# Pablete1234/parquet-floor

Measured on AMD Instinct MI355X. Metric: decoded GB/s + rows/s (node), lineitem-shape Snappy+dict, 1/2/4/8 GPUs, higher is better.
Workload: dtype u8; 1 GPU; lineitem SF1 x1 (6001215 rows x 1, 16 cols, 6 row groups of 1Mi rows), Snappy + dictionary, device-resident; row_groups_per_rank=6, compressed_page_bytes_rank0=217870360

## Files before the change

parquet-floor_amd/csrc/pf_internal.h:

```cpp
#pragma once
#include <stdint.h>

#ifdef __HIPCC__
#define PF_HD __host__ __device__
#else
#define PF_HD
#endif

namespace pf {

struct Int2 {
    int x, y;
};

struct PfOpts {
    int exec = 5;
    bool ba_fused = true;
    bool page_null = false;
    int null_stagger = 0;
    bool nest_timeout = false;
    uint32_t null_dcap = 0;
    unsigned debug_skip = 0;
    int force_serial = 0;
    int force_redo = 0;
    bool zc = true;
    bool dl_kernel = true;
    bool h2d_kernel = false;
    int h2d_grid = 256;
    bool dl_stream = true;
    bool dl_prio = false;
    bool debug_plan = false;
    int64_t nest_seg = 0;
    bool nest_seg_set = false;
    bool dbp_par = true;
    bool bloom_first = true;
    bool flat_dstr = true;
    int fix_shift = 1;
};

constexpr uint32_t FBLK = 4096;
constexpr uint32_t BA_TILE = 8192;
constexpr uint64_t BA_SHORT = 48;
constexpr uint32_t STICKY_DICT = 64u << 10;
constexpr uint32_t SNAP_RB = 128;
constexpr uint32_t SNAP_WIN = 64 * SNAP_RB;
constexpr uint32_t SNAP_WWORDS = SNAP_WIN / 32;
constexpr uint32_t SNAP_BLOCK = 65536;

struct SnapWin {
    uint32_t entry;
    uint32_t exit;
    uint32_t out;
    uint32_t flags;
};

struct SnapEnt {
    uint32_t pos;
    uint32_t out;
};
// ... 19 lines not shown
    uint8_t* ddst;
    uint32_t dlo;
    uint32_t dgran;
    uint32_t dflags;
    uint32_t lit;
};

struct ZstdJob {
    const uint8_t* src;
    uint8_t* dst;
    uint32_t src_len;
    uint32_t dst_len;
    int32_t page;
    int32_t chunk;
    uint32_t exact;
    uint32_t produced;
};
constexpr int ZSTD_GRID = 512;
constexpr uint32_t ZSTD_LIT_MAX = 128u << 10;
PF_HD inline uint32_t zstd_lit_stride(uint32_t max_dst) {
    return ((max_dst < ZSTD_LIT_MAX ? max_dst : ZSTD_LIT_MAX) + 255u) / 256u * 256u + 256u;
}

enum : int32_t { DONE_FIXED = 1, DONE_FLAT = 2, DONE_NULL = 4, DONE_PAGE = 8, DONE_DSTR = 16 };

enum : int32_t { DIRECT_NONE = 0, DIRECT_VALUES = 1, DIRECT_INPLACE = 2 };

struct DevPage {
    const uint8_t* body;
    const uint8_t* lvl;
    uint32_t body_len;
    uint32_t rep_len;
    uint32_t def_len;
    int32_t chunk;
    int32_t flags;
    int32_t encoding;
    int32_t def_enc;
    int32_t rep_enc;
    int32_t num_values;
    int32_t done;
    int64_t entry_start;
    int64_t n_slots;
    int64_t n_values;
    int64_t n_rows;
    int64_t n_chars;
    int64_t slot_start;
    int64_t value_start;
// ... 206 lines not shown
```

parquet-floor_amd/csrc/pf_launch.h:

```cpp
#pragma once
#include <hip/hip_runtime.h>

#include "pf_internal.h"
#include "pfloor.h"

namespace pf {

void launch_snappy_serial(const SnappyJob* d_jobs, int n_jobs, const int* d_fallback, DevChunkResult* d_res, hipStream_t s);
void launch_snappy_parse(const SnappyJob* d_jobs, int n_jobs, const int2* d_wins, int n_wins, SnapWin* d_win, SnapEnt* d_ent,
                         uint32_t* d_lane_out, uint32_t* d_splits, int* d_fb, int max_nwin, hipStream_t s);
void launch_snappy_exec(const SnappyJob* d_jobs, int n_jobs, const int2* d_pieces, int n_pieces, uint32_t* d_splits, int* d_fb,
                        DevChunkResult* d_res, int exec, hipStream_t s);
void launch_snappy(const SnappyJob* d_jobs, int n_jobs, const int2* d_wins, int n_wins, SnapWin* d_win, SnapEnt* d_ent,
                   uint32_t* d_lane_out, const int2* d_pieces, int n_pieces, uint32_t* d_splits, int* d_fb,
                   DevChunkResult* d_res, int max_nwin, int exec, hipStream_t s);

void launch_zstd(ZstdJob* d_jobs, const int* d_order, int n_jobs, uint8_t* d_lit, uint32_t lit_stride, DevChunkResult* d_res,
                 hipStream_t s);

void launch_snappy_head(SnappyJob* d_jobs, int n_jobs, DevPage* d_pages, const DevChunk* d_chunks, int* d_fb,
                        const DevChunkResult* d_res, hipStream_t st);
void launch_snappy_litcopy(const SnappyJob* d_jobs, const int* d_list, int n, const int* d_fb, hipStream_t st);

void launch_ba(BaJob* d_jobs, int n_jobs, const int2* d_tiles, int n_tiles, DevChunkResult* d_res, hipStream_t st,
               bool short_values);

void launch_runs(const DevChunk* d_chunks, DevPage* d_pages, const int* d_list, int n, DevChunkResult* d_res, hipStream_t st);
void launch_lvl(const DevChunk* d_chunks, DevPage* d_pages, const int* d_list, int n, DevChunkResult* d_res, hipStream_t st,
                bool page_null, NullCaps nc);
void launch_count_flat(const DevChunk* d_chunks, DevPage* d_pages, const int* d_list, int n, int n_flat, const int2* d_dblk,
                       int n_dblk, DevChunkResult* d_res, BaJob* d_bajobs, hipStream_t st);
void launch_flat(const DevChunk* d_chunks, DevPage* d_pages, const int* d_list, int nfix, int n, int n4, int n8, int* d_fbq,
                 const int2* d_dblk, int n_dblk, DevChunkResult* d_res, hipStream_t st, NullCaps nc, int stagger);

void launch_nest_lvl(const DevChunk* d_chunks, DevPage* d_pages, const int* d_list, int n, int max_nwin, DevChunkResult* d_res,
                     hipStream_t st, bool force_timeout);
void launch_count(const DevChunk* d_chunks, DevPage* d_pages, const int* d_list, int n, DevChunkResult* d_res, BaJob* d_bajobs,
                  hipStream_t st, int idle_grid);
void launch_nest_count(const DevChunk* d_chunks, DevPage* d_pages, const int* d_list, int n, const int2* d_segs, int n_segs,
                       DevChunkResult* d_res, hipStream_t st);
void launch_scan(DevChunk* d_chunks, DevPage* d_pages, const int* d_list, int n, DevChunkResult* d_res, uint8_t* arena,
                 uint64_t cap, unsigned long long* used, hipStream_t st);
void launch_decode(const DevChunk* d_chunks, DevPage* d_pages, const int* d_list, int n, int n_first, DevChunkResult* d_res,
                   hipStream_t st, int idle_grid);
void launch_nest_decode(const DevChunk* d_chunks, DevPage* d_pages, const int2* d_segs, int n_segs, DevChunkResult* d_res,
                        hipStream_t st);

void launch_delta(const DevChunk* d_chunks, DevPage* d_pages, const int* d_list, int n, int max_dbp_nwin, DevChunkResult* d_res,
                  hipStream_t st);
void launch_dlen(const DevChunk* d_chunks, DevPage* d_pages, const int* d_list, int n, DevChunkResult* d_res, hipStream_t st);
void launch_dba_chars(const DevChunk* d_chunks, DevPage* d_pages, const int* d_list, int n, DevChunkResult* d_res, hipStream_t st);

void launch_window(const DevChunk* d_chunks, const DevChunkResult* d_res, const DevWin* d_wins, DevWinRes* d_wres, int n_wins,
                   int copy_grid, const uint8_t* chars_base, uint8_t* wchars_base, int64_t out_delta, int64_t bits_delta,
                   hipStream_t st);

// ... 10 lines not shown
```

parquet-floor_amd/csrc/pf_pages.hip:

```cpp
#include <hip/hip_runtime.h>

#include "pf_dstr_ids.h"
#include "pf_launch.h"
#include "pf_pages.h"
#include "pf_snappy_par.h"

namespace pf {

#ifdef PF_STAMPS
__device__ unsigned long long pf_pstamps[16];
#define PSTAMP(i, v) atomicAdd(&pf_pstamps[i], (unsigned long long)(v))
extern "C" int pf_debug_pstamps(unsigned long long* out, int n, int reset) {
    if (hipMemcpyFromSymbol(out, HIP_SYMBOL(pf_pstamps), sizeof(unsigned long long) * (n < 16 ? n : 16)) != hipSuccess) return -1;
    if (reset) {
        unsigned long long z[16] = {};
        if (hipMemcpyToSymbol(HIP_SYMBOL(pf_pstamps), z, sizeof z) != hipSuccess) return -1;
    }
    return 0;
}
#else
#define PSTAMP(i, v) ((void)0)
#endif

#ifndef PF_FT
// ... 32 lines not shown
    }
    const uint32_t ne = uint32_t(pg.num_values);
    const int id_bw = int(s.val[0]);
    if (tid == 0) {
        s_allp = ck.max_def == 0 ? 1 : (s.def_rle ? all_present(s.def, s.def_n, bit_width(ck.max_def), ne, uint32_t(ck.max_def)) : 0);
    } else if (tid >= 64) {
        __shared__ RunWalk s_st;
        int nr = 0;
        uint32_t cov = 0;
        const int rr = wave_walk_runs(s.val + 1, s.val_n - 1, id_bw, 0, ne, R, RUN_CAP, nr, cov, s_st, RunWalk{0, 0});
        if (tid == 64) { s_res = rr; s_nr = nr; s_cov = cov; }
    }
    __syncthreads();
    const int nr = s_nr;
    if (s_res == 2) {
        if (tid == 0) { T[2] = 0; T[3] = 0; }
        return;
    }
    for (int i = tid; i < nr; i += 128) {
        T[4 + 2 * i] = R[i].first | (R[i].packed << 31);
        T[5 + 2 * i] = R[i].data;
    }
    if (tid == 0) { T[0] = uint32_t(nr); T[1] = s_cov; T[2] = 1u; T[3] = s_allp ? 1u : 0u; }
}

__device__ __forceinline__ bool count_dict_page(const DevPage& pg, const DevChunk& ck, const Sections& s) {
    const uint32_t* T = pg.runtab;
    return T != nullptr && T[3] == 1u && T[0] <= uint32_t(RUN_CAP) && T[1] >= uint32_t(pg.num_values) && ck.dict_len &&
           s.val_n > 0 && flat_block_chars(pg) != nullptr;
}
constexpr uint64_t BC_BAD = ~0ull;

__global__ __launch_bounds__(NT) void k_count_dict(const DevChunk* __restrict__ chunks, DevPage* pages,
                                                   const int2* __restrict__ blocks, DevChunkResult* res) {
    __shared__ Run R[RUN_CAP];
    __shared__ uint32_t s_len[DSTR_CAP];
    __shared__ unsigned long long s_acc;
    const int2 pb = blocks[blockIdx.x];
    DevPage& pg = pages[pb.x];
    const DevChunk& ck = chunks[pg.chunk];
    const int tid = threadIdx.x;
    if (res[pg.chunk].status != 0 || ck.max_rep != 0 || ck.ptype != 6 || !is_dict_enc(pg.encoding)) return;
    Sections s;
    if (!page_sections(pg, ck, s) || !count_dict_page(pg, ck, s)) return;
    const uint32_t ne = uint32_t(pg.num_values);
    const uint32_t b0 = uint32_t(pb.y) * FBLK;
// ... 544 lines not shown
                const uint32_t m = uint32_t((hi - lo >= 32 ? 0xffffffffull : ((1ull << (hi - lo)) - 1ull)) << (lo & 31));
                if (lo == (wd << 5) && hi == ((wd + 1) << 5)) vw[wd] = m;
                else atomicOr(vw + wd, m);
            }
        }
        if (__syncthreads_or(bad)) return 1;
    }
    return 0;
}

__device__ __forceinline__ bool flat_fixed_block(FixedLds& S, const DevChunk* __restrict__ chunks, DevPage* pages, const int2 pbk,
                                 DevChunkResult* res) {
    if (pbk.x < 0) return true;
    const int pi = pbk.x;
    const uint32_t blk = uint32_t(pbk.y) & 0x0fffffffu;
    const uint32_t bsz = FBLK << (uint32_t(pbk.y) >> 28);
    DevPage& pg = pages[pi];
    const DevChunk& ck = chunks[pg.chunk];
    const int tid = threadIdx.x;
    const int* jfb = pg.jfb;
    const bool dval = pg.direct == DIRECT_VALUES;
    const int jf = jfb != nullptr ? *jfb : FB_WHOLE + 1;
    const int done = pg.done;
    if (done & DONE_DSTR) return true;
    if ((res[pg.chunk].status != 0) | (ck.max_rep != 0) | (ck.ptype == 6) | ((done & DONE_NULL) != 0)) return false;
    if (dval & (jf <= FB_WHOLE)) {
        const uint32_t ne = uint32_t(pg.num_values), e_begin = blk * bsz;
        if (e_begin >= ne && blk > 0) return true;
        const uint32_t e_end = min(ne, e_begin + bsz);
        if (ck.max_def > 0 && ck.validity && e_end > e_begin) {
            const uint64_t b0 = uint64_t(pg.entry_start) + e_begin, b1 = uint64_t(pg.entry_start) + e_end;
            uint32_t* vw = reinterpret_cast<uint32_t*>(ck.validity);
            for (uint64_t wd = (b0 >> 5) + threadIdx.x; wd <= ((b1 - 1) >> 5); wd += NT) {
                const uint64_t lo = max(b0, wd << 5), hi = min(b1, (wd + 1) << 5);
                const uint32_t m = uint32_t((hi - lo >= 32 ? 0xffffffffull : ((1ull << (hi - lo)) - 1ull)) << (lo & 31));
                if (lo == (wd << 5) && hi == ((wd + 1) << 5)) vw[wd] = m;
                else atomicOr(vw + wd, m);
            }
        }
        if (threadIdx.x == 0) {
            if (ck.needs_count == 0)
                atomicAdd(reinterpret_cast<unsigned long long*>(&res[pg.chunk].num_values), (unsigned long long)(e_end - e_begin));
            atomicOr(&pg.done, DONE_FIXED);
        }
        return true;
    }
    Sections s;
// ... 406 lines not shown
struct DstrLds {
    uint32_t rt[2 * RUN_CAP];
    uint32_t dpl[DSTR_CAP];
    u32x4 dict[DSTR_DICT / 16 + 2];
    u32x4 win[DSTR_WIN / 16 + 2];
    uint32_t scan_tmp[NT / 64];
    uint32_t wlo[NT / 64], whi[NT / 64];
};
#ifdef PF_DIAG
__device__ unsigned long long pf_dstr_counts[2];
extern "C" int pf_debug_dstr_counts(unsigned long long* out, int reset) {
    if (hipMemcpyFromSymbol(out, HIP_SYMBOL(pf_dstr_counts), sizeof(unsigned long long) * 2) != hipSuccess) return -1;
    if (reset) {
        const unsigned long long z[2] = {0, 0};
        if (hipMemcpyToSymbol(HIP_SYMBOL(pf_dstr_counts), z, sizeof z) != hipSuccess) return -1;
    }
    return 0;
}
#define DSTR_COUNT(i) (threadIdx.x == 0 ? (void)atomicAdd(&pf_dstr_counts[i], 1ull) : (void)0)
#else
#define DSTR_COUNT(i) ((void)0)
#endif

__device__ __forceinline__ u32x4 ld16_within(uintptr_t a, uintptr_t beg, uintptr_t end) {
    if (a >= beg && a + 16u <= end) return *reinterpret_cast<const PF_GLOBAL u32x4*>(a);
    uint32_t q[4] = {0, 0, 0, 0};
    #pragma unroll
    for (uint32_t b = 0; b < 16u; b++)
        if (a + b >= beg && a + b < end) q[b >> 2] |= uint32_t(*reinterpret_cast<const PF_GLOBAL uint8_t*>(a + b)) << (8 * (b & 3));
    return u32x4{q[0], q[1], q[2], q[3]};
}

template <int LEAD>
__device__ __forceinline__ void store_offs16(int32_t* p, const uint32_t (&o)[16]) {
    #pragma unroll
    for (int k = 0; k < LEAD; k++) p[k] = int32_t(o[k]);
    #pragma unroll
    for (int k = LEAD; k + 4 <= 16; k += 4) *reinterpret_cast<u32x4*>(p + k) = u32x4{o[k], o[k + 1], o[k + 2], o[k + 3]};
    #pragma unroll
    for (int k = LEAD + (16 - LEAD) / 4 * 4; k < 16; k++) p[k] = int32_t(o[k]);
}

__global__ __launch_bounds__(NT, PF_DSTR_OCC) void k_flat_dstr(const DevChunk* __restrict__ chunks, DevPage* pages,
                                                            const int2* __restrict__ blocks, DevChunkResult* res) {
    __shared__ DstrLds S;
    const int2 pb = blocks[blockIdx.x];
    const int pi = pb.x;
    const uint32_t blk = uint32_t(pb.y);
    DevPage& pg = pages[pi];
    const DevChunk& ck = chunks[pg.chunk];
    const int tid = threadIdx.x;
    const uint32_t ne = uint32_t(pg.num_values);
    const uint32_t b0 = blk * FBLK;
    if (blk > 0 && b0 >= ne) return;
    bool ok = (res[pg.chunk].status == 0) & (ck.max_rep == 0) & (ck.ptype == 6) & is_dict_enc(pg.encoding) & (pg.counted == 1) &
// ... 8 lines not shown
        const DevPage& dp = pages[ck.dict_page];
        dend = reinterpret_cast<uintptr_t>(dp.body) + dp.body_len;
        ok = dend > dbeg && dend - dbeg <= uintptr_t(DSTR_DICT);
    }
    if (!ok) {
        if (blk == 0) DSTR_COUNT(1);
        return;
    }
    const uint32_t b1 = min(ne, b0 + FBLK);
    const uint32_t* T = pg.runtab;
    const uint32_t nr = T[0], cov = T[1];
    const uint32_t dn = uint32_t(ck.dict_n), dbytes = uint32_t(dend - dbeg);
    const int id_bw = int(s.val[0]);
    const uint8_t* ids = s.val + 1;
    const uint64_t ids_n = s.val_n - 1;
    const uint64_t bc_blk = blk > 0 ? flat_block_chars(pg)[blk] : 0ull;
    int bad = 0;
    uint32_t mylo = 0xffffffffu, myhi = 0u;
    if (uint32_t(tid) < nr) {
        const uint32_t f = T[4 + 2 * tid], d = T[5 + 2 * tid];
        const uint32_t nf = uint32_t(tid) + 1 < nr ? (T[6 + 2 * tid] & 0x7fffffffu) : cov;
        S.rt[2 * tid] = f;
        S.rt[2 * tid + 1] = d;
        const uint32_t first = f & 0x7fffffffu;
        const uint32_t a = max(first, b0), z = min(nf, b1);
        if ((f >> 31) && a < z) {
            mylo = uint32_t((uint64_t(d) + uint64_t(a - first) * uint64_t(id_bw)) >> 3);
            myhi = uint32_t((uint64_t(d) + uint64_t(z - first) * uint64_t(id_bw) + 7u) >> 3);
        }
    }
    const uint32_t doff = uint32_t(dbeg & 15u);
    if (uint32_t(tid) < dn) {
        const uint32_t pos = gptr(ck.dict_pos)[tid], len = gptr(ck.dict_len)[tid];
        bad = (len > DSTR_LMAX) | (pos > dbytes) | (len > dbytes - min(pos, dbytes));
        S.dpl[tid] = (doff + pos) | (len << 16);
    }
    for (uint32_t c = tid; c < (doff + dbytes + 15u) / 16u; c += NT) S.dict[c] = ld16_within(dbeg - doff + 16u * c, dbeg, dend);
    #pragma unroll
    for (int d = 32; d >= 1; d >>= 1) {
        mylo = min(mylo, uint32_t(__shfl_xor(mylo, d, 64)));
        myhi = max(myhi, uint32_t(__shfl_xor(myhi, d, 64)));
    }
    if ((tid & 63) == 0) { S.wlo[tid >> 6] = mylo; S.whi[tid >> 6] = myhi; }
    if (__syncthreads_or(bad)) {
        if (blk == 0) DSTR_COUNT(1);
        return;
    }
    uint32_t lo = 0xffffffffu, hi = 0u;
    #pragma unroll
    for (int w = 0; w < NT / 64; w++) { lo = min(lo, S.wlo[w]); hi = max(hi, S.whi[w]); }
    const uintptr_t ibeg = reinterpret_cast<uintptr_t>(ids), iend = ibeg + ids_n;
    const uintptr_t ia0 = (ibeg + (lo < hi ? lo : 0u)) & ~uintptr_t(15);
    const uint32_t inb = lo < hi ? (uint32_t(ibeg + hi - ia0) + 8u + 15u) & ~15u : 0u;
    const bool ilds = inb > 0 && inb <= uint32_t(sizeof(S.win));
    if (ilds) {
        for (uint32_t c = tid; c < inb / 16u; c += NT) S.win[c] = ld16_within(ia0 + 16u * c, ibeg, iend);
        __syncthreads();
    }
    const int64_t bias = ilds ? 8 * (int64_t(ibeg) - int64_t(ia0)) : 0;
    const uint32_t* const wl = reinterpret_cast<const uint32_t*>(S.win);
    const auto W = [&](uint32_t w) -> uint32_t {
        if (ilds) return wl[w];
        return ld32le(ids, uint64_t(w) * 4u, ids_n);
    };
    const uint32_t e0 = b0 + 16u * uint32_t(tid);
    const uint32_t n = e0 < b1 ? min(16u, b1 - e0) : 0u;
    uint32_t pl[16];
    uint32_t lsum = 0;
    {
        uint32_t id[16];
        dstr_ids16(S.rt, nr, cov, e0, n, id_bw, bias, W, id);
        #pragma unroll
        for (uint32_t k = 0; k < 16; k++) {
            pl[k] = 0;
            if (k >= n) continue;
            if (id[k] >= dn) { bad = 1; continue; }
            pl[k] = S.dpl[id[k]];
            lsum += pl[k] >> 16;
        }
    }
    uint32_t tot;
    const uint32_t lo_c = block_excl_scan<NT>(lsum, S.scan_tmp, tot);
// ... 48 lines not shown
            uint32_t v = my0;
            #pragma unroll
            for (uint32_t k = 0; k < 16; k++) {
                const uint32_t len = pl[k] >> 16, pos = pl[k] & 0xffffu;
                const uint32_t s0 = max(v, w0), s1 = min(v + len, w1);
                for (uint32_t b = s0; b < s1; b++) w8[b - w0] = d8[pos + (b - v)];
                v += len;
            }
        }
        __syncthreads();
        for (uint32_t ci = tid; ci < (w1 - w0 + 15u) / 16u; ci += NT) {
            const uint32_t vp = w0 + 16u * ci;
            if (vp >= a0c && vp + 16u <= vend) {
                *reinterpret_cast<PF_GLOBAL u32x4*>(g0 + vp) = S.win[ci];
            } else {
                for (uint32_t b = 0; b < 16u; b++)
                    if (vp + b >= a0c && vp + b < vend) reinterpret_cast<uint8_t*>(g0 + vp)[b] = w8[16u * ci + b];
            }
        }
    }
    if (tid == 0) {
        atomicOr(&pg.done, DONE_DSTR | DONE_FLAT);
        DSTR_COUNT(0);
    }
}

#ifndef PF_FLAT_OCC
#define PF_FLAT_OCC 5
#endif
__global__ __launch_bounds__(NT, PF_FLAT_OCC) void k_flat_all(const DevChunk* __restrict__ chunks, DevPage* pages,
                                                 const int2* __restrict__ blocks, int n, const int* __restrict__ fbq,
                                                 DevChunkResult* res) {
    __shared__ union FlatAllLds {
        FixedLds f;
        FlatLds g;
    } S;
    if (int(blockIdx.x) >= n) {
        const int nq = fbq[0], g = int(gridDim.x) - n;
        for (int i = int(blockIdx.x) - n; i < nq; i += g) {
            const int2 pq = reinterpret_cast<const int2*>(fbq + 4)[i];
            if (!flat_fixed_block(S.f, chunks, pages, pq, res)) {
                __syncthreads();
                flat_block(S.g, chunks, pages, pq, res);
            }
            __syncthreads();
        }
// ... 358 lines not shown

#ifndef PF_NTN
#define PF_NTN 256
#endif
constexpr int NTN = PF_NTN;
constexpr int NEPT = FBLK / NTN;
static_assert(NEPT % 4 == 0 && NEPT <= 16, "k_flat_null's stores and present masks");
struct NullLds {
    uint2 drun[LT_BLOCK_RUNS + 1];
    uint2 vrun[RUN_CAP + 1];
    uint32_t vbits[FBLK / 32 + 2];
    uint32_t scan_tmp[NTN / 64];
};
__device__ __forceinline__ uint32_t rl_first(uint2 r) { return r.x & 0x7fffffffu; }
__device__ __forceinline__ int rl_find(const uint2* runs, int nr, uint32_t i) {
    int lo = 0, hi = nr;
    while (hi - lo > 1) {
        const int mid = (lo + hi) >> 1;
        if (rl_first(runs[mid]) <= i) lo = mid; else hi = mid;
    }
    return lo;
}


template <int W> struct WidthType { using type = uint64_t; };
template <> struct WidthType<4> { using type = uint32_t; };

template <int W>
__global__ __launch_bounds__(NTN) void k_flat_null(const DevChunk* __restrict__ chunks, DevPage* pages,
                                                   const int2* __restrict__ blocks, DevChunkResult* res, NullCaps nc,
                                                   int stagger, int* fbq) {
    using VT = typename WidthType<W>::type;
    __shared__ __attribute__((aligned(16))) NullLds S;
    extern __shared__ __attribute__((aligned(16))) uint64_t DYN[];
    uint32_t* const s_dst = reinterpret_cast<uint32_t*>(DYN);
    uint32_t* const s_ist = s_dst + (nc.dcap + 32u) / 4u;
    uint64_t* const DL = reinterpret_cast<uint64_t*>(s_ist + (nc.icap + 32u) / 4u);
    const uint32_t dlds = nc.dlds;
    const int2 pbk = blocks[blockIdx.x];
#ifdef PF_DIAG
    if (stagger && pbk.y > 0)
        for (int i = 0; i < stagger; i++) __builtin_amdgcn_s_sleep(127);
#else
    (void)stagger;
#endif
    if (pbk.x < 0) return;
#ifdef PF_STAMPS
    unsigned long long t_ph = __builtin_amdgcn_s_memtime(), t_beg = t_ph;
#define NSTAMP(i) { const unsigned long long t_ = __builtin_amdgcn_s_memtime(); if (threadIdx.x == 0) PSTAMP(i, t_ - t_ph); t_ph = t_; }
// ... 565 lines not shown
#endif

void launch_count_flat(const DevChunk* d_chunks, DevPage* d_pages, const int* d_list, int n, int n_flat, const int2* d_dblk,
                       int n_dblk, DevChunkResult* d_res, BaJob* d_bajobs, hipStream_t st) {
    if (n <= 0) return;
    if (n_dblk > 0) hipLaunchKernelGGL(k_count_dict, dim3(n_dblk), dim3(NT), 0, st, d_chunks, d_pages, d_dblk, d_res);
    if (n_flat > 0) hipLaunchKernelGGL(k_count_flat, dim3(n_flat), dim3(NT), 0, st, d_chunks, d_pages, d_list, d_res, d_bajobs);
}
void launch_runs(const DevChunk* d_chunks, DevPage* d_pages, const int* d_list, int n, DevChunkResult* d_res,
                 hipStream_t st) {
    if (n > 0) hipLaunchKernelGGL(k_runs, dim3(n), dim3(128), 0, st, d_chunks, d_pages, d_list, d_res);
}
void launch_lvl(const DevChunk* d_chunks, DevPage* d_pages, const int* d_list, int n, DevChunkResult* d_res,
                hipStream_t st, bool page_null, NullCaps nc) {
    if (n <= 0) return;
#ifdef PF_DIAG
    if (page_null) hipLaunchKernelGGL(k_page_null, dim3(n), dim3(PN_NT), 0, st, d_chunks, d_pages, d_list, d_res);
#else
    (void)page_null;
#endif
    hipLaunchKernelGGL(k_lvl, dim3(n), dim3(LT_NT), 0, st, d_chunks, d_pages, d_list, d_res, nc.dcap, nc.icap);
}
void launch_flat(const DevChunk* d_chunks, DevPage* d_pages, const int* d_list, int nfix, int n, int n4, int n8, int* d_fbq,
                 const int2* d_dblk, int n_dblk, DevChunkResult* d_res, hipStream_t st, NullCaps nc, int stagger) {
    const int2* blocks = reinterpret_cast<const int2*>(d_list);
    const size_t dyn = size_t(nc.dcap) + 32u + nc.icap + 32u + nc.dlds;
    if (n4 > 0)
        hipLaunchKernelGGL(k_flat_null<4>, dim3(n4), dim3(NTN), dyn, st, d_chunks, d_pages, blocks + nfix + n, d_res, nc, stagger, d_fbq);
    if (n8 > 0)
        hipLaunchKernelGGL(k_flat_null<8>, dim3(n8), dim3(NTN), dyn, st, d_chunks, d_pages, blocks + nfix + n + n4, d_res, nc, stagger,
                           d_fbq);
    if (nfix > 0) hipLaunchKernelGGL(k_flat_fixed, dim3(nfix), dim3(NT), 0, st, d_chunks, d_pages, blocks, d_res, d_fbq);
    if (n_dblk > 0) hipLaunchKernelGGL(k_flat_dstr, dim3(n_dblk), dim3(NT), 0, st, d_chunks, d_pages, d_dblk, d_res);
    const int nq = nfix + n4 + n8;
    const int nqw = nq < 32 ? nq : 32;
    if (n + nqw > 0)
        hipLaunchKernelGGL(k_flat_all, dim3(n + nqw), dim3(NT), 0, st, d_chunks, d_pages, blocks + nfix, n, d_fbq, d_res);
}

}
```

parquet-floor_amd/csrc/pf_runtime.hip:

```cpp
#include <hip/hip_runtime.h>

#include <algorithm>
#include <chrono>
#include <cstdio>
#include <cstdlib>
#include <cstring>
#include <memory>
#include <mutex>
#include <string>
#include <vector>

#include "pf_ctx.h"
#include "pf_host.h"
#include "pf_launch.h"
#include "pf_plan.h"
#include "pf_snappy_par.h"
#include "pfloor.h"

using namespace pf;

static_assert(sizeof(Int2) == sizeof(int2) && alignof(Int2) <= alignof(int2), "the planner's pairs are the kernels' int2");

namespace {

// ... 112 lines not shown
    if (!(skip & 8u)) launch_runs(d_chunks, d_pages, list(L_RUNS), len(L_RUNS), d_res, st);
    NullCaps ncaps = p.null_caps;
    if (ctx->opts.null_dcap) ncaps.dcap = ctx->opts.null_dcap;
    if (!(skip & 8u)) launch_lvl(d_chunks, d_pages, list(L_LVL), len(L_LVL), d_res, st, ctx->opts.page_null, ncaps);
    launch_dlen(d_chunks, d_pages, list(L_DLEN), len(L_DLEN), d_res, st);
    EVREC(ctx, ctx->ev[6], st);
    launch_nest_lvl(d_chunks, d_pages, list(L_NEST), n_nest, p.max_nwin, d_res, st, ctx->opts.nest_timeout);
    if (!(skip & 16u)) {
        launch_count_flat(d_chunks, d_pages, list(L_COUNT), len(L_COUNT), p.n_count_flat, pairs(L_CDICT), len(L_CDICT) / 2,
                          d_res, d_bajobs, st);
        launch_count(d_chunks, d_pages, list(L_COUNT), len(L_COUNT), d_res, d_bajobs, st, COUNT_IDLE_GRID);
    }
    launch_nest_count(d_chunks, d_pages, list(L_NEST), n_nest, pairs(L_NSEG), n_nseg, d_res, st);
    if (!(skip & 4u))
        launch_ba(d_bajobs + p.n_ba_dict, n_ba - p.n_ba_dict, d_batiles + p.n_ba_dict_tiles, n_bt - p.n_ba_dict_tiles,
                  d_res, st, p.ba_short_data && ctx->opts.ba_fused);
    EVREC(ctx, ctx->ev[7], st);
    launch_scan(d_chunks, d_pages, list(L_SCAN), len(L_SCAN), d_res, static_cast<uint8_t*>(ctx->d_chars.p),
                ctx->d_chars.cap, used, st);
    EVREC(ctx, ctx->ev[8], st);
    if (!(skip & 32u))
        launch_flat(d_chunks, d_pages, list(L_FLAT), p.n_flat_fixed, p.n_flat_all, p.n_null4, p.n_null8,
                    reinterpret_cast<int*>(meta + p.off_nfbq), pairs(L_CDICT), ctx->opts.flat_dstr ? len(L_CDICT) / 2 : 0, d_res, st,
                    ncaps, ctx->opts.null_stagger);
    EVREC(ctx, ctx->ev[9], st);
    if (!(skip & 64u)) launch_decode(d_chunks, d_pages, list(L_DECODE), len(L_DECODE), p.n_decode_first, d_res, st, DECODE_IDLE_GRID);
    launch_nest_decode(d_chunks, d_pages, pairs(L_NSEG), n_nseg, d_res, st);
    launch_dba_chars(d_chunks, d_pages, list(L_DBA), len(L_DBA), d_res, st);
    EVREC(ctx, ctx->ev[10], st);
    const WinLayout& wl = ctx->win_lay;
    const bool windowed = !ctx->wins.empty();
    DevWinRes* d_wres = windowed ? reinterpret_cast<DevWinRes*>(static_cast<uint8_t*>(ctx->d_win.p) + wl.res_off) : nullptr;
    if (windowed) {
        EVREC(ctx, ctx->ev_win[0], st);
        launch_window(d_chunks, d_res, static_cast<DevWin*>(ctx->d_win.p), d_wres, int(ctx->wins.size()), ctx->win_grid,
                      static_cast<const uint8_t*>(ctx->d_chars.p), static_cast<uint8_t*>(ctx->d_wchars.p), ctx->twin.out,
                      ctx->twin.bits, st);
        EVREC(ctx, ctx->ev_win[1], st);
        HIPCHK(ctx, hipMemcpyAsync(static_cast<uint8_t*>(ctx->h_win.p) + wl.res_off, d_wres, wl.res_bytes, hipMemcpyDeviceToHost, st));
    }
    if (ctx->filtered()) {
        EVREC(ctx, ctx->ev_sel[0], st);
        launch_filter(d_chunks, d_res, d_wres, ctx->sel, ctx->n_chunks, ctx->sel_lay.grid, static_cast<const uint8_t*>(ctx->d_chars.p),
                      static_cast<uint8_t*>(ctx->d_wchars.p), ctx->twin.out, ctx->twin.bits, st);
        EVREC(ctx, ctx->ev_sel[1], st);
        HIPCHK(ctx, hipMemcpyAsync(ctx->h_sel.p, ctx->d_sel.p, ctx->sel_lay.o_up, hipMemcpyDeviceToHost, st));
    }
// ... 110 lines not shown
    o.null_dcap = uint32_t(std::max(0, num("PF_NULL_DCAP", 0))) & ~15u;
    o.null_stagger = num("PF_DEBUG_NULL_STAGGER", o.null_stagger);
    if (const char* e = std::getenv("PF_DEBUG_SKIP")) {
        const char* names[] = {"parse", "exec", "ba", "levels", "count", "flat", "decode"};
        for (int i = 0; i < 7; i++)
            if (std::strstr(e, names[i])) o.debug_skip |= 1u << i;
    }
    o.force_serial = num("PF_DEBUG_FORCE_SERIAL", o.force_serial);
    o.force_redo = num("PF_DEBUG_FORCE_REDO", o.force_redo);
    o.zc = on("PF_ZC", o.zc);
    o.dl_kernel = on("PF_DL_KERNEL", o.dl_kernel);
    o.dl_stream = on("PF_DL_STREAM", o.dl_stream);
    o.h2d_kernel = on("PF_H2D_KERNEL", o.h2d_kernel);
    o.h2d_grid = std::max(1, num("PF_H2D_GRID", o.h2d_grid));
    o.dl_prio = on("PF_DL_PRIO", o.dl_prio);
    o.debug_plan = on("PF_DEBUG_PLAN", o.debug_plan);
    if (const char* e = std::getenv("PF_NEST_SEG")) {
        o.nest_seg = std::atoll(e);
        o.nest_seg_set = true;
    }
    o.dbp_par = on("PF_DBP_PAR", o.dbp_par);
    o.bloom_first = on("PF_BLOOM_FIRST", o.bloom_first);
    o.flat_dstr = on("PF_FLAT_DSTR", o.flat_dstr);
    const int fb = num("PF_FIX_BLK", 8192);
    o.fix_shift = fb >= 16384 ? 2 : (fb >= 8192 ? 1 : 0);
}
#endif

int ctx_init(pf_ctx* ctx, pf_ctx* peer) {
#ifdef PF_DIAG
    opts_from_env(ctx->opts);
#endif
    HIPCHK(nullptr, hipSetDevice(ctx->device));
    if (peer) {
        ctx->streams = peer->streams;
    } else {
        ctx->streams = std::make_shared<Streams>();
        ctx->streams->device = ctx->device;
        HIPCHK(nullptr, hipStreamCreateWithFlags(&ctx->streams->stream, hipStreamNonBlocking));
    }
    ctx->stream = ctx->streams->stream;
    ctx->zc = ctx->opts.zc;
    HIPCHK(nullptr, hipEventCreateWithFlags(&ctx->ev_done, hipEventDisableTiming));
    HIPCHK(nullptr, hipEventCreateWithFlags(&ctx->ev_copy, hipEventDisableTiming));
    HIPCHK(nullptr, hipEventCreateWithFlags(&ctx->ev_dl, hipEventDisableTiming));
    for (auto& e : ctx->ev) HIPCHK(nullptr, hipEventCreate(&e));
// ... 777 lines not shown
```

Baseline: 392.9 decoded GB/s.

## Add dedicated dictionary-gather kernel for fixed-width dict pages using run tables

Adds k_flat_dfix, launched before k_flat_fixed, which decodes dictionary-encoded 4/8-byte fixed-width pages. It uses the precomputed run table, stages the dictionary and the needed slice of the id stream in LDS, gathers values and writes them with aligned 16-byte stores. Pages it finishes are marked DONE_DFIX so the generic fixed kernel skips them. The aim is to cut the global-memory gathers and scattered stores of the generic path. In exchange it adds another launch and an LDS footprint that may limit occupancy, and pages that fail its checks still fall back to the old path.

```diff
diff --git a/parquet-floor_amd/csrc/pf_internal.h b/parquet-floor_amd/csrc/pf_internal.h
--- a/parquet-floor_amd/csrc/pf_internal.h
+++ b/parquet-floor_amd/csrc/pf_internal.h
@@ -35,6 +35,7 @@
     bool dbp_par = true;
     bool bloom_first = true;
     bool flat_dstr = true;
+    bool flat_dfix = true;
     int fix_shift = 1;
 };
 
@@ -100,7 +101,7 @@
     return ((max_dst < ZSTD_LIT_MAX ? max_dst : ZSTD_LIT_MAX) + 255u) / 256u * 256u + 256u;
 }
 
-enum : int32_t { DONE_FIXED = 1, DONE_FLAT = 2, DONE_NULL = 4, DONE_PAGE = 8, DONE_DSTR = 16 };
+enum : int32_t { DONE_FIXED = 1, DONE_FLAT = 2, DONE_NULL = 4, DONE_PAGE = 8, DONE_DSTR = 16, DONE_DFIX = 32 };
 
 enum : int32_t { DIRECT_NONE = 0, DIRECT_VALUES = 1, DIRECT_INPLACE = 2 };
 
diff --git a/parquet-floor_amd/csrc/pf_launch.h b/parquet-floor_amd/csrc/pf_launch.h
--- a/parquet-floor_amd/csrc/pf_launch.h
+++ b/parquet-floor_amd/csrc/pf_launch.h
@@ -31,7 +31,8 @@
 void launch_count_flat(const DevChunk* d_chunks, DevPage* d_pages, const int* d_list, int n, int n_flat, const int2* d_dblk,
                        int n_dblk, DevChunkResult* d_res, BaJob* d_bajobs, hipStream_t st);
 void launch_flat(const DevChunk* d_chunks, DevPage* d_pages, const int* d_list, int nfix, int n, int n4, int n8, int* d_fbq,
-                 const int2* d_dblk, int n_dblk, DevChunkResult* d_res, hipStream_t st, NullCaps nc, int stagger);
+                 const int2* d_dblk, int n_dblk, DevChunkResult* d_res, hipStream_t st, NullCaps nc, int stagger,
+                 bool dfix);
 
 void launch_nest_lvl(const DevChunk* d_chunks, DevPage* d_pages, const int* d_list, int n, int max_nwin, DevChunkResult* d_res,
                      hipStream_t st, bool force_timeout);
diff --git a/parquet-floor_amd/csrc/pf_pages.hip b/parquet-floor_amd/csrc/pf_pages.hip
--- a/parquet-floor_amd/csrc/pf_pages.hip
+++ b/parquet-floor_amd/csrc/pf_pages.hip
@@ -78,6 +78,54 @@
         T[5 + 2 * i] = R[i].data;
     }
     if (tid == 0) { T[0] = uint32_t(nr); T[1] = s_cov; T[2] = 1u; T[3] = s_allp ? 1u : 0u; }
+}
+
+__device__ __forceinline__ u32x4 ld16_within(uintptr_t a, uintptr_t beg, uintptr_t end) {
+    if (a >= beg && a + 16u <= end) return *reinterpret_cast<const PF_GLOBAL u32x4*>(a);
+    uint32_t q[4] = {0, 0, 0, 0};
+    #pragma unroll
+    for (uint32_t b = 0; b < 16u; b++)
+        if (a + b >= beg && a + b < end) q[b >> 2] |= uint32_t(*reinterpret_cast<const PF_GLOBAL uint8_t*>(a + b)) << (8 * (b & 3));
+    return u32x4{q[0], q[1], q[2], q[3]};
+}
+
+__device__ __forceinline__ void run_id_bytes(uint32_t f, uint32_t d, uint32_t nf, uint32_t b0, uint32_t b1, int id_bw,
+                                             uint32_t& lo, uint32_t& hi) {
+    lo = 0xffffffffu;
+    hi = 0u;
+    const uint32_t first = f & 0x7fffffffu;
+    const uint32_t a = max(first, b0), z = min(nf, b1);
+    if ((f >> 31) && a < z) {
+        lo = uint32_t((uint64_t(d) + uint64_t(a - first) * uint64_t(id_bw)) >> 3);
+        hi = uint32_t((uint64_t(d) + uint64_t(z - first) * uint64_t(id_bw) + 7u) >> 3);
+    }
+}
+__device__ __forceinline__ void id_range_publish(uint32_t mylo, uint32_t myhi, uint32_t* wlo, uint32_t* whi) {
+    #pragma unroll
+    for (int d = 32; d >= 1; d >>= 1) {
+        mylo = min(mylo, uint32_t(__shfl_xor(mylo, d, 64)));
+        myhi = max(myhi, uint32_t(__shfl_xor(myhi, d, 64)));
+    }
+    if ((threadIdx.x & 63) == 0) { wlo[threadIdx.x >> 6] = mylo; whi[threadIdx.x >> 6] = myhi; }
+}
+enum : int { ID_NONE = 0, ID_STAGED = 1, ID_BIG = 2 };
+__device__ __forceinline__ int id_stage_load(u32x4* win, uint32_t cap, const uint32_t* wlo, const uint32_t* whi,
+                                              const uint8_t* ids, uint64_t ids_n, int64_t& bias) {
+    uint32_t lo = 0xffffffffu, hi = 0u;
+    #pragma unroll
+    for (int w = 0; w < NT / 64; w++) { lo = min(lo, wlo[w]); hi = max(hi, whi[w]); }
+    lo = __builtin_amdgcn_readfirstlane(lo);
+    hi = __builtin_amdgcn_readfirstlane(hi);
+    const uintptr_t ibeg = reinterpret_cast<uintptr_t>(ids), iend = ibeg + ids_n;
+    const uintptr_t ia0 = (ibeg + (lo < hi ? lo : 0u)) & ~uintptr_t(15);
+    const uint32_t inb = lo < hi ? (uint32_t(ibeg + hi - ia0) + 8u + 15u) & ~15u : 0u;
+    const bool ilds = inb > 0 && inb <= cap;
+    if (ilds) {
+        for (uint32_t c = threadIdx.x; c < inb / 16u; c += NT) win[c] = ld16_within(ia0 + 16u * c, ibeg, iend);
+        __syncthreads();
+    }
+    bias = ilds ? 8 * (int64_t(ibeg) - int64_t(ia0)) : 0;
+    return ilds ? ID_STAGED : (inb > 0 ? ID_BIG : ID_NONE);
 }
 
 __device__ __forceinline__ bool count_dict_page(const DevPage& pg, const DevChunk& ck, const Sections& s) {
@@ -668,7 +716,7 @@
     const bool dval = pg.direct == DIRECT_VALUES;
     const int jf = jfb != nullptr ? *jfb : FB_WHOLE + 1;
     const int done = pg.done;
-    if (done & DONE_DSTR) return true;
+    if (done & (DONE_DSTR | DONE_DFIX)) return true;
     if ((res[pg.chunk].status != 0) | (ck.max_rep != 0) | (ck.ptype == 6) | ((done & DONE_NULL) != 0)) return false;
     if (dval & (jf <= FB_WHOLE)) {
         const uint32_t ne = uint32_t(pg.num_values), e_begin = blk * bsz;
@@ -1121,15 +1169,6 @@
 #define DSTR_COUNT(i) ((void)0)
 #endif
 
-__device__ __forceinline__ u32x4 ld16_within(uintptr_t a, uintptr_t beg, uintptr_t end) {
-    if (a >= beg && a + 16u <= end) return *reinterpret_cast<const PF_GLOBAL u32x4*>(a);
-    uint32_t q[4] = {0, 0, 0, 0};
-    #pragma unroll
-    for (uint32_t b = 0; b < 16u; b++)
-        if (a + b >= beg && a + b < end) q[b >> 2] |= uint32_t(*reinterpret_cast<const PF_GLOBAL uint8_t*>(a + b)) << (8 * (b & 3));
-    return u32x4{q[0], q[1], q[2], q[3]};
-}
-
 template <int LEAD>
 __device__ __forceinline__ void store_offs16(int32_t* p, const uint32_t (&o)[16]) {
     #pragma unroll
@@ -1184,12 +1223,7 @@
         const uint32_t nf = uint32_t(tid) + 1 < nr ? (T[6 + 2 * tid] & 0x7fffffffu) : cov;
         S.rt[2 * tid] = f;
         S.rt[2 * tid + 1] = d;
-        const uint32_t first = f & 0x7fffffffu;
-        const uint32_t a = max(first, b0), z = min(nf, b1);
-        if ((f >> 31) && a < z) {
-            mylo = uint32_t((uint64_t(d) + uint64_t(a - first) * uint64_t(id_bw)) >> 3);
-            myhi = uint32_t((uint64_t(d) + uint64_t(z - first) * uint64_t(id_bw) + 7u) >> 3);
-        }
+        run_id_bytes(f, d, nf, b0, b1, id_bw, mylo, myhi);
     }
     const uint32_t doff = uint32_t(dbeg & 15u);
     if (uint32_t(tid) < dn) {
@@ -1198,28 +1232,13 @@
         S.dpl[tid] = (doff + pos) | (len << 16);
     }
     for (uint32_t c = tid; c < (doff + dbytes + 15u) / 16u; c += NT) S.dict[c] = ld16_within(dbeg - doff + 16u * c, dbeg, dend);
-    #pragma unroll
-    for (int d = 32; d >= 1; d >>= 1) {
-        mylo = min(mylo, uint32_t(__shfl_xor(mylo, d, 64)));
-        myhi = max(myhi, uint32_t(__shfl_xor(myhi, d, 64)));
-    }
-    if ((tid & 63) == 0) { S.wlo[tid >> 6] = mylo; S.whi[tid >> 6] = myhi; }
+    id_range_publish(mylo, myhi, S.wlo, S.whi);
     if (__syncthreads_or(bad)) {
         if (blk == 0) DSTR_COUNT(1);
         return;
     }
-    uint32_t lo = 0xffffffffu, hi = 0u;
-    #pragma unroll
-    for (int w = 0; w < NT / 64; w++) { lo = min(lo, S.wlo[w]); hi = max(hi, S.whi[w]); }
-    const uintptr_t ibeg = reinterpret_cast<uintptr_t>(ids), iend = ibeg + ids_n;
-    const uintptr_t ia0 = (ibeg + (lo < hi ? lo : 0u)) & ~uintptr_t(15);
-    const uint32_t inb = lo < hi ? (uint32_t(ibeg + hi - ia0) + 8u + 15u) & ~15u : 0u;
-    const bool ilds = inb > 0 && inb <= uint32_t(sizeof(S.win));
-    if (ilds) {
-        for (uint32_t c = tid; c < inb / 16u; c += NT) S.win[c] = ld16_within(ia0 + 16u * c, ibeg, iend);
-        __syncthreads();
-    }
-    const int64_t bias = ilds ? 8 * (int64_t(ibeg) - int64_t(ia0)) : 0;
+    int64_t bias;
+    const bool ilds = id_stage_load(S.win, uint32_t(sizeof(S.win)), S.wlo, S.whi, ids, ids_n, bias) == ID_STAGED;
     const uint32_t* const wl = reinterpret_cast<const uint32_t*>(S.win);
     const auto W = [&](uint32_t w) -> uint32_t {
         if (ilds) return wl[w];
@@ -1314,6 +1333,221 @@
     if (tid == 0) {
         atomicOr(&pg.done, DONE_DSTR | DONE_FLAT);
         DSTR_COUNT(0);
+    }
+}
+
+#ifndef PF_DFIX_LDS
+#define PF_DFIX_LDS 20480
+#endif
+#ifndef PF_DFIX_OCC
+#define PF_DFIX_OCC 5
+#endif
+#ifndef PF_DFIX_H4
+#define PF_DFIX_H4 8
+#endif
+#ifndef PF_DFIX_H8
+#define PF_DFIX_H8 4
+#endif
+static_assert(16 % PF_DFIX_H4 == 0 && PF_DFIX_H4 % 4 == 0 && 16 % PF_DFIX_H8 == 0 && PF_DFIX_H8 % 2 == 0, "whole 16-byte stores");
+constexpr uint32_t DFIX_LDS = PF_DFIX_LDS;
+static_assert(DFIX_LDS % 16 == 0 && DFIX_LDS >= 1024, "the id stage starts 16-byte aligned behind the dictionary");
+static_assert(RT_CAP >= uint32_t(NT) + 1u && RUN_CAP <= NT, "a thread a run row, read before the run count is known");
+struct DfixLds {
+    uint32_t rt[2 * RUN_CAP];
+    u32x4 reg[DFIX_LDS / 16 + 2];
+    uint32_t wlo[NT / 64], whi[NT / 64];
+};
+#ifdef PF_DIAG
+__device__ unsigned long long pf_dfix_counts[2];
+extern "C" int pf_debug_dfix_counts(unsigned long long* out, int reset) {
+    if (hipMemcpyFromSymbol(out, HIP_SYMBOL(pf_dfix_counts), sizeof(unsigned long long) * 2) != hipSuccess) return -1;
+    if (reset) {
+        const unsigned long long z[2] = {0, 0};
+        if (hipMemcpyToSymbol(HIP_SYMBOL(pf_dfix_counts), z, sizeof z) != hipSuccess) return -1;
+    }
+    return 0;
+}
+#define DFIX_COUNT(i) (threadIdx.x == 0 ? (void)atomicAdd(&pf_dfix_counts[i], 1ull) : (void)0)
+#else
+#define DFIX_COUNT(i) ((void)0)
+#endif
+
+template <int W> struct WidthType { using type = uint64_t; };
+template <> struct WidthType<4> { using type = uint32_t; };
+
+template <int LEAD, class VT, int N>
+__device__ __forceinline__ void store_vals(PF_GLOBAL VT* p, const VT (&v)[N]) {
+    constexpr int Q = 16 / int(sizeof(VT));
+    #pragma unroll
+    for (int k = 0; k < LEAD; k++) p[k] = v[k];
+    #pragma unroll
+    for (int k = LEAD; k + Q <= N; k += Q) {
+        u32x4 x;
+        if constexpr (sizeof(VT) == 4) x = u32x4{uint32_t(v[k]), uint32_t(v[k + 1]), uint32_t(v[k + 2]), uint32_t(v[k + 3])};
+        else x = u32x4{uint32_t(v[k]), uint32_t(uint64_t(v[k]) >> 32), uint32_t(v[k + 1]), uint32_t(uint64_t(v[k + 1]) >> 32)};
+        *reinterpret_cast<PF_GLOBAL u32x4*>(p + k) = x;
+    }
+    #pragma unroll
+    for (int k = LEAD + (N - LEAD) / Q * Q; k < N; k++) p[k] = v[k];
+}
+
+template <int W>
+__device__ __forceinline__ int dfix_body(DfixLds& S, const DevChunk& ck, const DevPage& pg, const Sections& s,
+                                         uint32_t e_begin, uint32_t e_end, uint32_t nr, uint32_t cov, uint32_t rf, uint32_t rd,
+                                         uint32_t rn) {
+    using VT = typename WidthType<W>::type;
+    constexpr int Q = 16 / W;
+    constexpr int H = W == 8 ? PF_DFIX_H8 : PF_DFIX_H4;
+    const int tid = threadIdx.x;
+    const uint64_t dn = uint64_t(ck.dict_n);
+    const int id_bw = int(s.val[0]);
+    const uint8_t* ids = s.val + 1;
+    const uint64_t ids_n = s.val_n - 1;
+    const PF_GLOBAL VT* gd = (const PF_GLOBAL VT*)(ck.dict_data);
+    const bool dlds = dn * uint64_t(W) <= uint64_t(DFIX_LDS);
+    const uint32_t dbytes = dlds ? (uint32_t(dn) * uint32_t(W) + 15u) & ~15u : 0u;
+    const bool row = uint32_t(tid) < nr;
+    {
+        uint32_t mylo = 0xffffffffu, myhi = 0u;
+        if (row) {
+            S.rt[2 * tid] = rf;
+            S.rt[2 * tid + 1] = rd;
+            run_id_bytes(rf, rd, uint32_t(tid) + 1 < nr ? (rn & 0x7fffffffu) : cov, e_begin, e_end, id_bw, mylo, myhi);
+        }
+        id_range_publish(mylo, myhi, S.wlo, S.whi);
+    }
+    VT* const sd = reinterpret_cast<VT*>(S.reg);
+    if (dlds) {
+        const uint32_t n32 = uint32_t(dn);
+        for (uint32_t i0 = tid; i0 < n32; i0 += 8u * NT) {
+            VT v[8];
+            #pragma unroll
+            for (uint32_t k = 0; k < 8; k++) v[k] = i0 + k * NT < n32 ? gd[i0 + k * NT] : VT(0);
+            #pragma unroll
+            for (uint32_t k = 0; k < 8; k++) if (i0 + k * NT < n32) sd[i0 + k * NT] = v[k];
+        }
+    }
+    u32x4* const stage = S.reg + dbytes / 16u;
+    const uint32_t cap = uint32_t(sizeof(S.reg)) - dbytes;
+    const uint32_t* const wl = reinterpret_cast<const uint32_t*>(stage);
+    const uint64_t slot_base = uint64_t(pg.entry_start);
+    __syncthreads();
+    int64_t bias;
+    int staged = id_stage_load(stage, cap, S.wlo, S.whi, ids, ids_n, bias);
+    const bool by_sub = staged == ID_BIG && e_end - e_begin > FBLK;
+    for (uint32_t b0 = e_begin; b0 < e_end; b0 += FBLK) {
+        const uint32_t b1 = min(e_end, b0 + FBLK);
+        if (by_sub) {
+            if (b0 == e_begin) __syncthreads();
+            uint32_t mylo = 0xffffffffu, myhi = 0u;
+            if (row) {
+                const uint32_t rnf = uint32_t(tid) + 1 < nr ? (S.rt[2 * tid + 2] & 0x7fffffffu) : cov;
+                run_id_bytes(S.rt[2 * tid], S.rt[2 * tid + 1], rnf, b0, b1, id_bw, mylo, myhi);
+            }
+            id_range_publish(mylo, myhi, S.wlo, S.whi);
+            __syncthreads();
+            staged = id_stage_load(stage, cap, S.wlo, S.whi, ids, ids_n, bias);
+        }
+        const bool ilds = staged == ID_STAGED;
+        const auto Wd = [&](uint32_t w) -> uint32_t {
+            if (ilds) return wl[w];
+            return ld32le(ids, uint64_t(w) * 4u, ids_n);
+        };
+        int bad = 0;
+        const uint32_t e0 = b0 + 16u * uint32_t(tid);
+        const uint32_t n = e0 < b1 ? min(16u, b1 - e0) : 0u;
+        if (n > 0) {
+            uint32_t id[16];
+            dstr_ids16(S.rt, nr, cov, e0, n, id_bw, bias, Wd, id);
+            #pragma unroll
+            for (uint32_t k = 0; k < 16; k++) {
+                if (uint64_t(id[k]) >= dn) { bad = 1; id[k] = 0u; }
+            }
+            PF_GLOBAL VT* const out = (PF_GLOBAL VT*)(ck.values) + (slot_base + e0);
+            const uint32_t lead = (uint32_t(16u - uint32_t(reinterpret_cast<uintptr_t>(out) & 15u)) & 15u) / uint32_t(W);
+            #pragma unroll
+            for (int h = 0; h < 16; h += H) {
+                VT v[H];
+                if (dlds) {
+                    #pragma unroll
+                    for (int k = 0; k < H; k++) v[k] = sd[id[h + k]];
+                } else {
+                    #pragma unroll
+                    for (int k = 0; k < H; k++) v[k] = gd[id[h + k]];
+                }
+                if (n == 16) {
+                    if constexpr (Q == 4) {
+                        switch (lead) {
+                            case 0: store_vals<0>(out + h, v); break;
+                            case 1: store_vals<1>(out + h, v); break;
+                            case 2: store_vals<2>(out + h, v); break;
+                            default: store_vals<3>(out + h, v); break;
+                        }
+                    } else {
+                        if (lead == 0) store_vals<0>(out + h, v);
+                        else store_vals<1>(out + h, v);
+                    }
+                } else {
+                    #pragma unroll
+                    for (int k = 0; k < H; k++) if (uint32_t(h + k) < n) out[h + k] = v[k];
+                }
+            }
+        }
+        if (ck.max_def > 0 && ck.validity) {
+            const uint64_t v0 = slot_base + b0, v1 = slot_base + b1;
+            uint32_t* vw = reinterpret_cast<uint32_t*>(ck.validity);
+            for (uint64_t wd = (v0 >> 5) + tid; wd <= ((v1 - 1) >> 5); wd += NT) {
+                const uint64_t l = max(v0, wd << 5), h = min(v1, (wd + 1) << 5);
+                const uint32_t m = uint32_t((h - l >= 32 ? 0xffffffffull : ((1ull << (h - l)) - 1ull)) << (l & 31));
+                if (l == (wd << 5) && h == ((wd + 1) << 5)) vw[wd] = m;
+                else atomicOr(vw + wd, m);
+            }
+        }
+        if (__syncthreads_or(bad)) return 1;
+    }
+    return 0;
+}
+
+__global__ __launch_bounds__(NT, PF_DFIX_OCC) void k_flat_dfix(const DevChunk* __restrict__ chunks, DevPage* pages,
+                                                            const int2* __restrict__ blocks, DevChunkResult* res) {
+    __shared__ DfixLds S;
+    const int2 pbk = blocks[blockIdx.x];
+    if (pbk.x < 0) return;
+    const int pi = pbk.x;
+    const uint32_t blk = uint32_t(pbk.y) & 0x0fffffffu;
+    const uint32_t bsz = FBLK << (uint32_t(pbk.y) >> 28);
+    DevPage& pg = pages[pi];
+    const DevChunk& ck = chunks[pg.chunk];
+    const uint32_t ne = uint32_t(pg.num_values);
+    const uint32_t e_begin = blk * bsz;
+    if (blk > 0 && e_begin >= ne) return;
+    const int w = ck.width;
+    bool ok = (res[pg.chunk].status == 0) & (ck.max_rep == 0) & (ck.ptype != 6) & (ck.ptype != 0) & ((w == 4) | (w == 8)) &
+              is_dict_enc(pg.encoding) & (ck.dict_data != nullptr) & (ck.dict_n > 0) & (pg.num_values > 0) &
+              ((pg.done & DONE_NULL) == 0) & (pg.direct != DIRECT_VALUES) & (pg.runtab != nullptr);
+    ok = ok && (reinterpret_cast<uintptr_t>(ck.dict_data) & uintptr_t(w - 1)) == 0;
+    const uint32_t* T = pg.runtab;
+    uint32_t t0 = 0, t1 = 0, t3 = 0, rf = 0, rd = 0, rn = 0;
+    if (ok) {
+        t0 = T[0]; t1 = T[1]; t3 = T[3];
+        rf = T[4 + 2 * threadIdx.x]; rd = T[5 + 2 * threadIdx.x]; rn = T[6 + 2 * threadIdx.x];
+    }
+    Sections s;
+    ok = ok && page_sections(pg, ck, s) && s.val_n > 0 && s.val[0] <= 32;
+    ok = ok && ((t3 == 1u) & (t0 <= uint32_t(RUN_CAP)) & (t1 >= ne));
+    if (!ok) {
+        if (blk == 0) DFIX_COUNT(1);
+        return;
+    }
+    const uint32_t e_end = min(ne, e_begin + bsz);
+    const int err = w == 4 ? dfix_body<4>(S, ck, pg, s, e_begin, e_end, t0, t1, rf, rd, rn)
+                           : dfix_body<8>(S, ck, pg, s, e_begin, e_end, t0, t1, rf, rd, rn);
+    if (threadIdx.x == 0) {
+        if (err) set_status(res, pg.chunk, ST_CORRUPT, pi);
+        else if (ck.needs_count == 0)
+            atomicAdd(reinterpret_cast<unsigned long long*>(&res[pg.chunk].num_values), (unsigned long long)(e_end - e_begin));
+        atomicOr(&pg.done, DONE_FIXED | DONE_DFIX);
+        DFIX_COUNT(0);
     }
 }
 
@@ -1718,9 +1952,6 @@
     return lo;
 }
 
-
-template <int W> struct WidthType { using type = uint64_t; };
-template <> struct WidthType<4> { using type = uint32_t; };
 
 template <int W>
 __global__ __launch_bounds__(NTN) void k_flat_null(const DevChunk* __restrict__ chunks, DevPage* pages,
@@ -2332,7 +2563,7 @@
     hipLaunchKernelGGL(k_lvl, dim3(n), dim3(LT_NT), 0, st, d_chunks, d_pages, d_list, d_res, nc.dcap, nc.icap);
 }
 void launch_flat(const DevChunk* d_chunks, DevPage* d_pages, const int* d_list, int nfix, int n, int n4, int n8, int* d_fbq,
-                 const int2* d_dblk, int n_dblk, DevChunkResult* d_res, hipStream_t st, NullCaps nc, int stagger) {
+                 const int2* d_dblk, int n_dblk, DevChunkResult* d_res, hipStream_t st, NullCaps nc, int stagger, bool dfix) {
     const int2* blocks = reinterpret_cast<const int2*>(d_list);
     const size_t dyn = size_t(nc.dcap) + 32u + nc.icap + 32u + nc.dlds;
     if (n4 > 0)
@@ -2340,6 +2571,7 @@
     if (n8 > 0)
         hipLaunchKernelGGL(k_flat_null<8>, dim3(n8), dim3(NTN), dyn, st, d_chunks, d_pages, blocks + nfix + n + n4, d_res, nc, stagger,
                            d_fbq);
+    if (nfix > 0 && dfix) hipLaunchKernelGGL(k_flat_dfix, dim3(nfix), dim3(NT), 0, st, d_chunks, d_pages, blocks, d_res);
     if (nfix > 0) hipLaunchKernelGGL(k_flat_fixed, dim3(nfix), dim3(NT), 0, st, d_chunks, d_pages, blocks, d_res, d_fbq);
     if (n_dblk > 0) hipLaunchKernelGGL(k_flat_dstr, dim3(n_dblk), dim3(NT), 0, st, d_chunks, d_pages, d_dblk, d_res);
     const int nq = nfix + n4 + n8;
diff --git a/parquet-floor_amd/csrc/pf_runtime.hip b/parquet-floor_amd/csrc/pf_runtime.hip
--- a/parquet-floor_amd/csrc/pf_runtime.hip
+++ b/parquet-floor_amd/csrc/pf_runtime.hip
@@ -158,7 +158,7 @@
     if (!(skip & 32u))
         launch_flat(d_chunks, d_pages, list(L_FLAT), p.n_flat_fixed, p.n_flat_all, p.n_null4, p.n_null8,
                     reinterpret_cast<int*>(meta + p.off_nfbq), pairs(L_CDICT), ctx->opts.flat_dstr ? len(L_CDICT) / 2 : 0, d_res, st,
-                    ncaps, ctx->opts.null_stagger);
+                    ncaps, ctx->opts.null_stagger, ctx->opts.flat_dfix && len(L_RUNS) > 0);
     EVREC(ctx, ctx->ev[9], st);
     if (!(skip & 64u)) launch_decode(d_chunks, d_pages, list(L_DECODE), len(L_DECODE), p.n_decode_first, d_res, st, DECODE_IDLE_GRID);
     launch_nest_decode(d_chunks, d_pages, pairs(L_NSEG), n_nseg, d_res, st);
@@ -315,6 +315,7 @@
     o.dbp_par = on("PF_DBP_PAR", o.dbp_par);
     o.bloom_first = on("PF_BLOOM_FIRST", o.bloom_first);
     o.flat_dstr = on("PF_FLAT_DSTR", o.flat_dstr);
+    o.flat_dfix = on("PF_FLAT_DFIX", o.flat_dfix);
     const int fb = num("PF_FIX_BLK", 8192);
     o.fix_shift = fb >= 16384 ? 2 : (fb >= 8192 ? 1 : 0);
 }
```

After: 394.7 decoded GB/s (median of 3 runs). Within noise of the previous version (+0.5%).
